# vseib/point-cloud-donkey

Measured on AMD Instinct MI355X. Metric: objects/sec classified (ModelNet10-like, SHOT-352), higher is better.
Workload: dtype f32; 1 GPU; configs[1]: ModelNet10-like test split, 16384 pts, 1024 uniform keypoints/object, SHOT-352 (Radius 0.4, LRF 0.3), exact kNN K=1 squared-L2, mean-shift bandwidth 0.6; points_per_object=16384, keypoints_per_object=1024, classes=10, codebook_words=102400, descriptor_dim=352, collective_world_size=1

## Files before the change

point-cloud-donkey_amd/csrc/knn_ring16.hip:

```cpp
#include "knn_internal.h"

namespace {

__device__ __forceinline__ void lds_dma16(const void* g, void* l) {
    __builtin_amdgcn_global_load_lds((const void __attribute__((address_space(1)))*)g, (void __attribute__((address_space(3)))*)l, 16, 0, 0);
}
template <int T, int WR = 2, int QP = 0, int PRE = 0>
__global__ __launch_bounds__(WR * 256, 2) void k_knn_l2_ring16(const u16* __restrict__ wh, const float* __restrict__ word_norm, int n_tiles_m, int ld, int k_steps,
                                                          const u16* __restrict__ qh, int nq, const float* __restrict__ out_scale,
                                                          int tiles_per_split, int n_splits,
                                                          float* __restrict__ cand_val, int* __restrict__ cand_idx, int cand_stride,
                                                          float* __restrict__ cand_bound, int bound_stride, unsigned int* __restrict__ stream_clock,
                                                          const float* __restrict__ thr_init, float* __restrict__ thr_out, int tile_step, float thr_relax) {
    using L = Ring16Lds<WR, QP>;
    constexpr int WC = 4, MT = 8, NT = 4, KB = RG_KB, BM = WR * 128, BN = RG_BN;
    constexpr int STAGES = L::STAGES, STAGE_HALVES = L::STAGE_HALVES, CNS = 256;
    extern __shared__ __attribute__((aligned(16))) unsigned char knn_smem[];
    u16* ring = (u16*)knn_smem;
    float* sCn = (float*)(knn_smem + L::cn);
    float* sThr = (float*)(knn_smem + L::thr);
    u16* panel = (u16*)(knn_smem + L::panel);
    const float oscale = out_scale[0];

    const int tid = threadIdx.x;
    const int lane = tid & 63;
    const int wv = __builtin_amdgcn_readfirstlane(tid >> 6);
    const int wr = wv / WC, wc = wv % WC;
    const int fr = lane & 15, fq = lane >> 4;
    const int xcd = blockIdx.x & 7, jx = blockIdx.x >> 3;
    const int split = jx % n_splits, qtile = (jx / n_splits) * 8 + xcd;
    if (qtile * BN >= nq) return;
    const int mt0 = split * tiles_per_split;
    const int n_t = PRE ? (n_tiles_m + tile_step - 1) / tile_step : min(n_tiles_m, mt0 + tiles_per_split) - mt0;
    if (n_t <= 0) return;
    const int nk = (k_steps + 1) / 2;
    const int G = n_t * nk;
    int toff = 0; unsigned c0 = 0u;
    if (stream_clock) {
        unsigned int* clk = stream_clock + xcd * n_splits + split;
        if (tid == 0) *(volatile unsigned*)ring = __hip_atomic_load(clk, __ATOMIC_RELAXED, __HIP_MEMORY_SCOPE_AGENT);
        __syncthreads();
        c0 = __builtin_amdgcn_readfirstlane(*(volatile unsigned*)ring);
        __syncthreads();
        toff = (int)(c0 % (unsigned)n_t);
        stream_clock = clk;
    }
    auto tile_of = [&](int i) { if (PRE) return i * tile_step; const int x = i + toff; return mt0 + (x >= n_t ? x - n_t : x); };

    constexpr int NA = QP ? 2 : (WR == 2 ? 4 : 2), NB = 4;
    const bool dma_a = QP || WR == 1 || wv < 4, dma_b = !QP && (WR == 1 || wv >= 4);
    const unsigned lane_off = (unsigned)(lane * 16);
    const int row_a = QP ? wv * 32 : (WR == 2 ? (wv & 3) * 64 : wv * 32), row_b = (wv & 3) * 64;
    const char* qbase = QP ? (const char*)(qh + (size_t)qtile * nk * (256 * KB)) + (wv * 32) * (KB * 2)
                           : (const char*)(qh + (size_t)qtile * nk * (BN * KB)) + row_b * (KB * 2);
    if (QP) {
        for (int s_ = 0; s_ < nk; ++s_) {
            lds_dma16(qbase + (size_t)s_ * (256 * KB * 2) + lane_off, panel + (s_ * 256 + wv * 32) * KB);
            lds_dma16(qbase + (size_t)s_ * (256 * KB * 2) + 16 * KB * 2 + lane_off, panel + (s_ * 256 + wv * 32 + 16) * KB);
        }
    }
    int pt = 0, pkc = 0, ps = 0;
    auto issue = [&]() {
        u16* st = ring + ps * STAGE_HALVES;
        const int tt = tile_of(pt);
        if (wv == 0 && pkc == 0) lds_dma16(word_norm + (size_t)tt * BM + lane * 4, sCn + (pt & 3) * CNS);
        if (dma_a) {
            const char* sp = (const char*)wh + ((size_t)(WR == 2 ? tt : (tt >> 1)) * nk + pkc) * (256 * KB * 2) + ((WR == 2 ? 0 : (tt & 1) * 128) + row_a) * (KB * 2);
#pragma unroll
            for (int j = 0; j < NA; ++j) lds_dma16(sp + j * (16 * KB * 2) + lane_off, st + (row_a + j * 16) * KB);
        }
        if (dma_b) {
            const char* sp = qbase + (size_t)pkc * (BN * KB * 2);
#pragma unroll
            for (int j = 0; j < NB; ++j) lds_dma16(sp + j * (16 * KB * 2) + lane_off, st + BM * KB + (row_b + j * 16) * KB);
        }
        if (++ps == STAGES) ps = 0;
        if (pt * nk + pkc + 1 < G) { if (++pkc == nk) { pkc = 0; ++pt; } }
    };
#pragma unroll
    for (int i = 0; i < STAGES; ++i) issue();

    const int fso = (fr * KB) + ((fq ^ f16t_swizzle(fr)) << 3);
    const int fragA = wr * (MT * 16) * KB + fso, fragB = (QP ? 0 : BM * KB) + wc * (NT * 16) * KB + fso;
    TopT<T + 1> top[NT];
    float thr[NT];
#pragma unroll
    for (int n = 0; n < NT; ++n) {
        top[n].init(); thr[n] = -__builtin_inff();
        if (!PRE && thr_init) { const int qi_ = qtile * BN + wc * (NT * 16) + n * 16 + fr; if (qi_ < nq) thr[n] = thr_init[qi_]; }
    }
    f32x4 acc[MT][NT];
    const int pw = (1 - wr) * WC + wc;
    if (WR == 2) {
#pragma unroll
        for (int n = 0; n < NT; ++n) sThr[(wv * NT + n) * 64 + lane] = -__builtin_inff();
    }

    f16x8 xa[4], ya[4], bq[NT];
    if (QP) asm volatile("s_waitcnt vmcnt(6)\n\ts_barrier" ::: "memory");
    else asm volatile("s_waitcnt vmcnt(12)\n\ts_barrier" ::: "memory");
#pragma unroll
    for (int m = 0; m < 4; ++m) xa[m] = *(const f16x8*)(ring + fragA + m * 16 * KB);
    int t = 0, kc = 0, gs = 0;
    for (int g = 0; g < G; ++g) {
        const int gn = gs + 1 == STAGES ? 0 : gs + 1;
        const u16* st = ring + gs * STAGE_HALVES;
        const u16* sn = ring + gn * STAGE_HALVES;
        gs = gn;
#pragma unroll
        for (int n = 0; n < NT; ++n) bq[n] = *(const f16x8*)((QP ? panel + kc * (256 * KB) : st) + fragB + n * 16 * KB);
        __builtin_amdgcn_sched_barrier(0);
        __builtin_amdgcn_s_setprio(1);
        const float* cnp = sCn + (t & 3) * CNS + wr * (MT * 16) + 4 * fq;
        auto mma4 = [&](int mb, const f16x8* af, f16x8* nxt, const u16* nsrc) {
            if (kc == 0) {
#pragma unroll
                for (int mt = 0; mt < 4; ++mt) {
                    const f32x4 c0 = *(const f32x4*)(cnp + (mb + mt) * 16);
#pragma unroll
                    for (int nt = 0; nt < NT; ++nt) acc[mb + mt][nt] = __builtin_amdgcn_mfma_f32_16x16x32_f16(af[mt], bq[nt], c0, 0, 0, 0);
                    nxt[mt] = *(const f16x8*)(nsrc + mt * 16 * KB);
                    __builtin_amdgcn_sched_barrier(0);
                }
            } else {
#pragma unroll
                for (int mt = 0; mt < 4; ++mt) {
#pragma unroll
                    for (int nt = 0; nt < NT; ++nt) acc[mb + mt][nt] = __builtin_amdgcn_mfma_f32_16x16x32_f16(af[mt], bq[nt], acc[mb + mt][nt], 0, 0, 0);
                    nxt[mt] = *(const f16x8*)(nsrc + mt * 16 * KB);
                    __builtin_amdgcn_sched_barrier(0);
                }
            }
        };
        mma4(0, xa, ya, st + fragA + 4 * 16 * KB);
        __builtin_amdgcn_sched_barrier(0);
        if (QP) asm volatile("s_waitcnt vmcnt(4) lgkmcnt(0)\n\ts_barrier" ::: "memory");
        else if (WR == 2) asm volatile("s_waitcnt vmcnt(8) lgkmcnt(0)\n\ts_barrier" ::: "memory");
        else asm volatile("s_waitcnt vmcnt(6) lgkmcnt(0)\n\ts_barrier" ::: "memory");
        issue();
        __builtin_amdgcn_sched_barrier(0);
        mma4(4, ya, xa, sn + fragA);
        __builtin_amdgcn_s_setprio(0);
        __builtin_amdgcn_sched_barrier(0);
        if (++kc == nk) {
            const int row0 = tile_of(t) * BM + wr * (MT * 16) + 4 * fq;
            if (stream_clock && tid == 0) atomicMax(stream_clock, c0 + (unsigned)t + 1u);
            if (PRE) {
#pragma unroll
                for (int nt = 0; nt < NT; ++nt) {
                    float m = thr[nt];
#pragma unroll
                    for (int mt = 0; mt < MT; ++mt) {
                        asm("v_max3_f32 %0, %1, %2, %3" : "=v"(m) : "v"(m), "v"(acc[mt][nt][0]), "v"(acc[mt][nt][1]));
                        asm("v_max3_f32 %0, %1, %2, %3" : "=v"(m) : "v"(m), "v"(acc[mt][nt][2]), "v"(acc[mt][nt][3]));
                    }
                    thr[nt] = m;
                }
            } else {
                float mx[NT];
#pragma unroll
                for (int nt = 0; nt < NT; ++nt) {
                    float m;
                    asm("v_max3_f32 %0, %1, %2, %3" : "=v"(m) : "v"(acc[0][nt][0]), "v"(acc[0][nt][1]), "v"(acc[0][nt][2]));
                    asm("v_max_f32 %0, %1, %2" : "=v"(m) : "v"(m), "v"(acc[0][nt][3]));
#pragma unroll
                    for (int mt = 1; mt < MT; ++mt) {
                        asm("v_max3_f32 %0, %1, %2, %3" : "=v"(m) : "v"(m), "v"(acc[mt][nt][0]), "v"(acc[mt][nt][1]));
                        asm("v_max3_f32 %0, %1, %2, %3" : "=v"(m) : "v"(m), "v"(acc[mt][nt][2]), "v"(acc[mt][nt][3]));
                    }
                    mx[nt] = m;
                }
                unsigned long long hit[NT];
#pragma unroll
                for (int nt = 0; nt < NT; ++nt) hit[nt] = __ballot(mx[nt] > thr[nt]);
                unsigned long long any_hit = 0ull;
#pragma unroll
                for (int nt = 0; nt < NT; ++nt) any_hit |= hit[nt];
                if (__builtin_expect(any_hit != 0ull, 0)) {
#pragma unroll
                    for (int nt = 0; nt < NT; ++nt) {
                        if (hit[nt] == 0ull) continue;
                        float gm[MT];
#pragma unroll
                        for (int mt = 0; mt < MT; ++mt) {
                            asm("v_max3_f32 %0, %1, %2, %3" : "=v"(gm[mt]) : "v"(acc[mt][nt][0]), "v"(acc[mt][nt][1]), "v"(acc[mt][nt][2]));
                            asm("v_max_f32 %0, %1, %2" : "=v"(gm[mt]) : "v"(gm[mt]), "v"(acc[mt][nt][3]));
                        }
                        unsigned long long gk[MT];
#pragma unroll
                        for (int mt = 0; mt < MT; ++mt) gk[mt] = __ballot(gm[mt] > thr[nt]);
                        asm volatile("" :: "s"(gk[0]), "s"(gk[1]), "s"(gk[2]), "s"(gk[3]), "s"(gk[4]), "s"(gk[5]), "s"(gk[6]), "s"(gk[7]));
#pragma unroll
                        for (int mt = 0; mt < MT; ++mt) {
                            if (gk[mt] == 0ull) continue;
                            unsigned long long mk[4];
#pragma unroll
                            for (int j = 0; j < 4; ++j) mk[j] = __ballot(acc[mt][nt][j] > thr[nt]);
                            asm volatile("" :: "s"(mk[0]), "s"(mk[1]), "s"(mk[2]), "s"(mk[3]));
#pragma unroll
                            for (int j = 0; j < 4; ++j) {
                                if (mk[j] == 0ull) continue;
                                const float a = acc[mt][nt][j];
                                top[nt].push_flat(a > thr[nt] ? -a : __builtin_inff(), row0 + mt * 16 + j);
                                asm("v_max_f32_e64 %0, %1, -%2" : "=v"(thr[nt]) : "v"(thr[nt]), "v"(top[nt].v[T]));
                            }
                        }
                    }
                }
            }
#pragma unroll
            for (int nt = 0; nt < NT; ++nt) {
                const auto h = __builtin_amdgcn_permlane32_swap(__float_as_uint(thr[nt]), __float_as_uint(thr[nt]), false, false);
                float sh;
                asm("v_max_f32 %0, %1, %2" : "=v"(sh) : "v"(__uint_as_float(h[0])), "v"(__uint_as_float(h[1])));
                const auto q = __builtin_amdgcn_permlane16_swap(__float_as_uint(sh), __float_as_uint(sh), false, false);
                asm("v_max_f32 %0, %1, %2" : "=v"(sh) : "v"(__uint_as_float(q[0])), "v"(__uint_as_float(q[1])));
                if (WR == 2) {
                    sThr[(wv * NT + nt) * 64 + lane] = sh;
                    const float other = sThr[(pw * NT + nt) * 64 + lane];
                    asm("v_max_f32 %0, %1, %2" : "=v"(thr[nt]) : "v"(sh), "v"(other));
                } else thr[nt] = sh;
            }
            kc = 0; ++t;
        }
    }
    asm volatile("s_waitcnt vmcnt(0)" ::: "memory");
    if (PRE) {
        __syncthreads();
#pragma unroll
        for (int nt = 0; nt < NT; ++nt) sThr[(wv * NT + nt) * 64 + lane] = thr[nt];
        __syncthreads();
        if (wr == 0 && fq == 0) {
#pragma unroll
            for (int nt = 0; nt < NT; ++nt) {
                const int qi = qtile * BN + wc * (NT * 16) + nt * 16 + fr;
                const float b = fmaxf(thr[nt], sThr[(pw * NT + nt) * 64 + lane]);
                if (qi < nq) thr_out[qi] = b - fabsf(b) * 3.814697265625e-06f + thr_relax;
            }
        }
        return;
    }
    if (WR == 2) {
        __syncthreads();
#pragma unroll
        for (int nt = 0; nt < NT; ++nt) sThr[(wv * NT + nt) * 64 + lane] = thr[nt];
        __syncthreads();
#pragma unroll
        for (int nt = 0; nt < NT; ++nt) thr[nt] = fmaxf(thr[nt], sThr[(pw * NT + nt) * 64 + lane]);
    }
#pragma unroll
    for (int nt = 0; nt < NT; ++nt) {
        const int qi = qtile * BN + wc * (NT * 16) + nt * 16 + fr;
        if (qi < nq) {
#pragma unroll
            for (int tt = 0; tt < T; ++tt) {
                const size_t o = (size_t)qi * cand_stride + split * (WR * 4 * T) + (wr * 4 + fq) * T + tt;
                cand_val[o] = -oscale * top[nt].v[tt]; cand_idx[o] = top[nt].i[tt];
            }
            cand_bound[(size_t)qi * bound_stride + split * (WR * 4) + (wr * 4 + fq)] = oscale * thr[nt];
        }
    }
}

template <int T>
const void* ring16_instance(int WR, int QP, int PRE) {
    if (PRE) return (const void*)k_knn_l2_ring16<T, 2, 0, 1>;
    if (WR == 1) return (const void*)k_knn_l2_ring16<T, 1>;
    return QP ? (const void*)k_knn_l2_ring16<T, 2, 2> : (const void*)k_knn_l2_ring16<T, 2>;
}

}

const void* knn_ring16_kernel(int T, int WR, int QP, int PRE) {
    switch (T) {
    case 1: return ring16_instance<1>(WR, QP, PRE);
    case 2: return ring16_instance<2>(WR, QP, PRE);
    case 3: return ring16_instance<3>(WR, QP, PRE);
    case 4: return ring16_instance<4>(WR, QP, PRE);
    }
    return nullptr;
}

int knn_ring16_launch(ismhip_ctx* ctx, int T, const void* kern, unsigned grid, int threads, size_t lds, KnnCandArgs a,
                      unsigned int* stream_clock, float* thr0, int pre_step, float pre_relax) {
    const float* thr_init = nullptr; float* thr_out = nullptr; int tile_step = 1;
    if (thr0 && pre_step > 0) {
        const void* pk = knn_ring16_kernel(T, 2, 0, 1);
        const size_t plds = Ring16Lds<2, 0>::total(0);
        const int rc2 = ism_lds_cap(ctx, pk, plds);
        if (rc2 != ISMHIP_OK) return rc2;
        int one = 1, all = a.n_tiles_m; unsigned int* noclk = nullptr; const float* noinit = nullptr;
        void* pargs[] = {&a.wh, &a.word_norm, &a.n_tiles_m, &a.ld, &a.k_steps, &a.qh, &a.nq, &a.out_scale, &all, &one, &a.cand_val, &a.cand_idx, &a.cand_stride, &a.cand_bound, &a.bound_stride, &noclk, &noinit, &thr0, &pre_step, &pre_relax};
        ISM_HIP(ctx, hipLaunchKernel(pk, dim3(grid / a.n_splits), dim3(512), pargs, plds, ctx->stream));
        ISM_CHECK_LAUNCH(ctx, "k_knn_l2_ring16<pre>");
    }
    thr_init = thr0;
    float no_relax = 0.f;
    void* rargs[] = {&a.wh, &a.word_norm, &a.n_tiles_m, &a.ld, &a.k_steps, &a.qh, &a.nq, &a.out_scale, &a.tiles_per_split, &a.n_splits, &a.cand_val, &a.cand_idx, &a.cand_stride, &a.cand_bound, &a.bound_stride, &stream_clock, &thr_init, &thr_out, &tile_step, &no_relax};
    ISM_HIP(ctx, hipLaunchKernel(kern, dim3(grid), dim3(threads), rargs, lds, ctx->stream));
    ISM_CHECK_LAUNCH(ctx, "k_knn_l2_ring16");
    return ISMHIP_OK;
}
```

Measured before the change: 18550 objects/s.

## Move threshold reduction and LDS exchange into hit path; lean top-k walk for small T

The per-tile cross-lane threshold reduction (permlane swaps) and the LDS exchange with the partner wave now run only when a tile actually has candidate hits, instead of after every tile. The partner threshold is read from LDS at the start of each epilogue. For small T, per-group maxima are computed once and reused in the hit path, and top-k insertion uses a branchless cndmask-based push. This is meant to cut per-tile epilogue overhead in the common no-hit case. The cost is possibly staler thresholds, which lead to more false hits, plus extra registers for the cached group maxima. The PRE path now reduces across lanes only once, at the end.

```diff
diff --git a/point-cloud-donkey_amd/csrc/knn_ring16.hip b/point-cloud-donkey_amd/csrc/knn_ring16.hip
--- a/point-cloud-donkey_amd/csrc/knn_ring16.hip
+++ b/point-cloud-donkey_amd/csrc/knn_ring16.hip
@@ -4,6 +4,29 @@
 
 __device__ __forceinline__ void lds_dma16(const void* g, void* l) {
     __builtin_amdgcn_global_load_lds((const void __attribute__((address_space(1)))*)g, (void __attribute__((address_space(3)))*)l, 16, 0, 0);
+}
+__device__ __forceinline__ float max_of_row_groups(float x) {
+    const auto h = __builtin_amdgcn_permlane32_swap(__float_as_uint(x), __float_as_uint(x), false, false);
+    float sh;
+    asm("v_max_f32 %0, %1, %2" : "=v"(sh) : "v"(__uint_as_float(h[0])), "v"(__uint_as_float(h[1])));
+    const auto q = __builtin_amdgcn_permlane16_swap(__float_as_uint(sh), __float_as_uint(sh), false, false);
+    asm("v_max_f32 %0, %1, %2" : "=v"(sh) : "v"(__uint_as_float(q[0])), "v"(__uint_as_float(q[1])));
+    return sh;
+}
+__device__ __forceinline__ float sel_f(unsigned long long m, float t, float f) { float r; asm("v_cndmask_b32_e64 %0, %1, %2, %3" : "=v"(r) : "v"(f), "v"(t), "s"(m)); return r; }
+__device__ __forceinline__ int sel_i(unsigned long long m, int t, int f) { int r; asm("v_cndmask_b32_e64 %0, %1, %2, %3" : "=v"(r) : "v"(f), "v"(t), "s"(m)); return r; }
+template <int N>
+__device__ __forceinline__ void push_cnd(TopT<N>& tp, float x, int idx) {
+    unsigned long long c[N];
+#pragma unroll
+    for (int t = 0; t < N; ++t) asm("v_cmp_lt_f32_e64 %0, %1, %2" : "=s"(c[t]) : "v"(x), "v"(tp.v[t]));
+#pragma unroll
+    for (int t = N - 1; t > 0; --t) {
+        tp.v[t] = sel_f(c[t - 1], tp.v[t - 1], sel_f(c[t], x, tp.v[t]));
+        tp.i[t] = sel_i(c[t - 1], tp.i[t - 1], sel_i(c[t], idx, tp.i[t]));
+    }
+    tp.v[0] = sel_f(c[0], x, tp.v[0]);
+    tp.i[0] = sel_i(c[0], idx, tp.i[0]);
 }
 template <int T, int WR = 2, int QP = 0, int PRE = 0>
 __global__ __launch_bounds__(WR * 256, 2) void k_knn_l2_ring16(const u16* __restrict__ wh, const float* __restrict__ word_norm, int n_tiles_m, int ld, int k_steps,
@@ -15,6 +38,7 @@
     using L = Ring16Lds<WR, QP>;
     constexpr int WC = 4, MT = 8, NT = 4, KB = RG_KB, BM = WR * 128, BN = RG_BN;
     constexpr int STAGES = L::STAGES, STAGE_HALVES = L::STAGE_HALVES, CNS = 256;
+    constexpr bool LEAN_WALK = T <= 3;
     extern __shared__ __attribute__((aligned(16))) unsigned char knn_smem[];
     u16* ring = (u16*)knn_smem;
     float* sCn = (float*)(knn_smem + L::cn);
@@ -157,38 +181,63 @@
                     thr[nt] = m;
                 }
             } else {
-                float mx[NT];
+                float other[NT];
+                if (WR == 2) {
+#pragma unroll
+                    for (int nt = 0; nt < NT; ++nt) other[nt] = sThr[(pw * NT + nt) * 64 + lane];
+                    __builtin_amdgcn_sched_barrier(0);
+                }
+                float gm[LEAN_WALK ? NT : 1][MT], mx[NT];
 #pragma unroll
                 for (int nt = 0; nt < NT; ++nt) {
                     float m;
-                    asm("v_max3_f32 %0, %1, %2, %3" : "=v"(m) : "v"(acc[0][nt][0]), "v"(acc[0][nt][1]), "v"(acc[0][nt][2]));
-                    asm("v_max_f32 %0, %1, %2" : "=v"(m) : "v"(m), "v"(acc[0][nt][3]));
-#pragma unroll
-                    for (int mt = 1; mt < MT; ++mt) {
-                        asm("v_max3_f32 %0, %1, %2, %3" : "=v"(m) : "v"(m), "v"(acc[mt][nt][0]), "v"(acc[mt][nt][1]));
-                        asm("v_max3_f32 %0, %1, %2, %3" : "=v"(m) : "v"(m), "v"(acc[mt][nt][2]), "v"(acc[mt][nt][3]));
+                    if (LEAN_WALK) {
+#pragma unroll
+                        for (int mt = 0; mt < MT; ++mt) {
+                            asm("v_max3_f32 %0, %1, %2, %3" : "=v"(gm[nt][mt]) : "v"(acc[mt][nt][0]), "v"(acc[mt][nt][1]), "v"(acc[mt][nt][2]));
+                            asm("v_max_f32 %0, %1, %2" : "=v"(gm[nt][mt]) : "v"(gm[nt][mt]), "v"(acc[mt][nt][3]));
+                        }
+                        asm("v_max3_f32 %0, %1, %2, %3" : "=v"(m) : "v"(gm[nt][0]), "v"(gm[nt][1]), "v"(gm[nt][2]));
+                        asm("v_max3_f32 %0, %1, %2, %3" : "=v"(m) : "v"(m), "v"(gm[nt][3]), "v"(gm[nt][4]));
+                        asm("v_max3_f32 %0, %1, %2, %3" : "=v"(m) : "v"(m), "v"(gm[nt][5]), "v"(gm[nt][6]));
+                        asm("v_max_f32 %0, %1, %2" : "=v"(m) : "v"(m), "v"(gm[nt][7]));
+                    } else {
+                        asm("v_max3_f32 %0, %1, %2, %3" : "=v"(m) : "v"(acc[0][nt][0]), "v"(acc[0][nt][1]), "v"(acc[0][nt][2]));
+                        asm("v_max_f32 %0, %1, %2" : "=v"(m) : "v"(m), "v"(acc[0][nt][3]));
+#pragma unroll
+                        for (int mt = 1; mt < MT; ++mt) {
+                            asm("v_max3_f32 %0, %1, %2, %3" : "=v"(m) : "v"(m), "v"(acc[mt][nt][0]), "v"(acc[mt][nt][1]));
+                            asm("v_max3_f32 %0, %1, %2, %3" : "=v"(m) : "v"(m), "v"(acc[mt][nt][2]), "v"(acc[mt][nt][3]));
+                        }
                     }
                     mx[nt] = m;
                 }
+                if (WR == 2) {
+#pragma unroll
+                    for (int nt = 0; nt < NT; ++nt) asm("v_max_f32 %0, %1, %2" : "=v"(thr[nt]) : "v"(thr[nt]), "v"(other[nt]));
+                }
                 unsigned long long hit[NT];
 #pragma unroll
                 for (int nt = 0; nt < NT; ++nt) hit[nt] = __ballot(mx[nt] > thr[nt]);
                 unsigned long long any_hit = 0ull;
 #pragma unroll
                 for (int nt = 0; nt < NT; ++nt) any_hit |= hit[nt];
-                if (__builtin_expect(any_hit != 0ull, 0)) {
+                if (any_hit != 0ull) {
 #pragma unroll
                     for (int nt = 0; nt < NT; ++nt) {
                         if (hit[nt] == 0ull) continue;
-                        float gm[MT];
+                        float gl[MT];
 #pragma unroll
                         for (int mt = 0; mt < MT; ++mt) {
-                            asm("v_max3_f32 %0, %1, %2, %3" : "=v"(gm[mt]) : "v"(acc[mt][nt][0]), "v"(acc[mt][nt][1]), "v"(acc[mt][nt][2]));
-                            asm("v_max_f32 %0, %1, %2" : "=v"(gm[mt]) : "v"(gm[mt]), "v"(acc[mt][nt][3]));
+                            if (LEAN_WALK) gl[mt] = gm[nt][mt];
+                            else {
+                                asm("v_max3_f32 %0, %1, %2, %3" : "=v"(gl[mt]) : "v"(acc[mt][nt][0]), "v"(acc[mt][nt][1]), "v"(acc[mt][nt][2]));
+                                asm("v_max_f32 %0, %1, %2" : "=v"(gl[mt]) : "v"(gl[mt]), "v"(acc[mt][nt][3]));
+                            }
                         }
                         unsigned long long gk[MT];
 #pragma unroll
-                        for (int mt = 0; mt < MT; ++mt) gk[mt] = __ballot(gm[mt] > thr[nt]);
+                        for (int mt = 0; mt < MT; ++mt) gk[mt] = __ballot(gl[mt] > thr[nt]);
                         asm volatile("" :: "s"(gk[0]), "s"(gk[1]), "s"(gk[2]), "s"(gk[3]), "s"(gk[4]), "s"(gk[5]), "s"(gk[6]), "s"(gk[7]));
 #pragma unroll
                         for (int mt = 0; mt < MT; ++mt) {
@@ -201,31 +250,23 @@
                             for (int j = 0; j < 4; ++j) {
                                 if (mk[j] == 0ull) continue;
                                 const float a = acc[mt][nt][j];
-                                top[nt].push_flat(a > thr[nt] ? -a : __builtin_inff(), row0 + mt * 16 + j);
+                                const float x = a > thr[nt] ? -a : __builtin_inff();
+                                if (LEAN_WALK) push_cnd(top[nt], x, row0 + mt * 16 + j); else top[nt].push_flat(x, row0 + mt * 16 + j);
                                 asm("v_max_f32_e64 %0, %1, -%2" : "=v"(thr[nt]) : "v"(thr[nt]), "v"(top[nt].v[T]));
                             }
                         }
+                        thr[nt] = max_of_row_groups(thr[nt]);
+                        if (WR == 2) sThr[(wv * NT + nt) * 64 + lane] = thr[nt];
                     }
                 }
-            }
-#pragma unroll
-            for (int nt = 0; nt < NT; ++nt) {
-                const auto h = __builtin_amdgcn_permlane32_swap(__float_as_uint(thr[nt]), __float_as_uint(thr[nt]), false, false);
-                float sh;
-                asm("v_max_f32 %0, %1, %2" : "=v"(sh) : "v"(__uint_as_float(h[0])), "v"(__uint_as_float(h[1])));
-                const auto q = __builtin_amdgcn_permlane16_swap(__float_as_uint(sh), __float_as_uint(sh), false, false);
-                asm("v_max_f32 %0, %1, %2" : "=v"(sh) : "v"(__uint_as_float(q[0])), "v"(__uint_as_float(q[1])));
-                if (WR == 2) {
-                    sThr[(wv * NT + nt) * 64 + lane] = sh;
-                    const float other = sThr[(pw * NT + nt) * 64 + lane];
-                    asm("v_max_f32 %0, %1, %2" : "=v"(thr[nt]) : "v"(sh), "v"(other));
-                } else thr[nt] = sh;
             }
             kc = 0; ++t;
         }
     }
     asm volatile("s_waitcnt vmcnt(0)" ::: "memory");
     if (PRE) {
+#pragma unroll
+        for (int nt = 0; nt < NT; ++nt) thr[nt] = max_of_row_groups(thr[nt]);
         __syncthreads();
 #pragma unroll
         for (int nt = 0; nt < NT; ++nt) sThr[(wv * NT + nt) * 64 + lane] = thr[nt];
```

Measured after the change: 18760 objects/s, median of 6. +1.1%, better.
